# hangelwen/miR-PREFeR

Hardware: AMD Instinct MI355X
Metric: precursor windows folded+filtered/sec (L=300) (higher is better)
Workload: dtype int16/int32 (energies in 0.01 kcal/mol)

## Files before the change

mir-prefer_amd/csrc/fold_lds_common.h:

```cpp
#pragma once
#include <hip/hip_runtime.h>
#include <type_traits>
#include <cstdio>
#include "fold_epilogue.h"
#include "fold185_device.h"

namespace mirp {

#define LNT 1024
#define LNT2 512
#define LCAP 352
#define LDMAX 300
#define LSPAN 300
#define I16_INF 0x7fff
#define FIN_LIMIT 28000
#define FML_BIAS 31500
#define FML_MAX 1267
#define LSEG 384
#define KEY_BIAS 40000
#define KEY_NONE 0xffffffffu
#define KEY_INF (65535u << 10)
#define OTH_BIAS 2048

struct LdsTables {
    short stack[64];
    short bulge[32];
    short internal_loop[32];
    short mismatchI[200], mismatchH[200], mismatchM[200], mismatch1nI[200], mismatch23I[200];
    unsigned char XB[176];
    unsigned char X1[176];
    short dangle5[40], dangle3[40];
    unsigned char rt2[28];
    short ML_closing, ML_intern, TerminalAU, ninio, MAX_NINIO, pad[3];
};
__host__ __device__ constexpr int xt_pslot(int s) { return s == 3 ? 3 : s == 4 ? 4 : 0; }
__host__ __device__ constexpr int xt_qslot(int s) { return s == 1 ? 1 : s == 3 ? 2 : s == 4 ? 1 : 0; }
__host__ __device__ constexpr int xt_pcode(int sp, int sp_m1) { return xt_pslot(sp) * 25 + sp_m1; }
__host__ __device__ constexpr int xt_qcode(int sq, int sq_p1) { return xt_qslot(sq) * 25 + sq_p1 * 5; }
static_assert(xt_pslot(1) + xt_qslot(4) == 1 && xt_pslot(2) + xt_qslot(3) == 2 && xt_pslot(3) + xt_qslot(2) == 3 && xt_pslot(3) + xt_qslot(4) == 4 &&
              xt_pslot(4) + xt_qslot(1) == 5 && xt_pslot(4) + xt_qslot(3) == 6, "inner-pair table slots");
template <class TAB>
__device__ inline void xt_fill(TAB& T, const FoldParams* __restrict__ P, int tid, int nt) {
    for (int x = tid; x < 175; x += nt) {
        const int slot = x / 25, a = (x % 25) / 5, b = x % 5;
        const int sp = slot == 1 ? 1 : slot == 2 ? 2 : (slot == 3 || slot == 4) ? 3 : 4, sq = slot == 1 ? 4 : slot == 2 ? 3 : slot == 3 ? 2 : slot == 4 ? 4 : slot == 5 ? 1 : 3;
        const int t2 = slot ? rtype_of(pair_type(sp, sq)) : 0;
        int xb = 0, x1 = 0;
        if (t2) {
            const int mi = P->mismatchI[t2][a][b];
            xb = (t2 > 2 ? P->TerminalAU : 0) - mi;
            x1 = P->mismatch1nI[t2][a][b] - mi;
        }
        T.XB[x] = (unsigned char)(xb + P->xb_bias); T.X1[x] = (unsigned char)(x1 + P->x1_bias);
    }
}
#define CSTR 354
static_assert(CSTR == MIRP_RING_CSTR, "FoldParams::ring_rowoff is built for this row stride");
#define MIRP_CK(d) ((d) % 3)
#define CRING_ROWS 33

struct LTab {
    static constexpr bool kTiled = true;
    const short* fml;
    const int* off;
    const short* carch;
    const unsigned short* tb;
    __device__ __forceinline__ int at(int d, int i) const { return off[(i - 1) >> 3] + ((i - 1) & 7) + 8 * (d - 4); }
    __device__ __forceinline__ int TB(int d, int i) const { return tb[at(d, i)]; }
    __device__ __forceinline__ int C(int d, int i) const { int v = carch[at(d, i)]; return v == I16_INF ? INF : v; }
    __device__ __forceinline__ int TBat(int o) const { return tb[o]; }
    __device__ __forceinline__ int Cat(int o) const { int v = carch[o]; return v == I16_INF ? INF : v; }
    __device__ __forceinline__ int Mat(int o) const { const int v = (unsigned short)fml[o]; return v == 65535 ? INF : v - FML_BIAS; }
    __device__ __forceinline__ int M(int d, int i) const {
        if (d < 4) return INF;
        const int v = (unsigned short)fml[at(d, i)];
        return v == 65535 ? INF : v - FML_BIAS;
    }
};

__device__ __forceinline__ int lds_mlstem(const LdsTables& T, const FoldParams* __restrict__ P, int type, int a, int b) {
    int e = T.ML_intern + (type > 2 ? T.TerminalAU : 0);
    if (a >= 0 && b >= 0) e += T.mismatchM[type * 25 + a * 5 + b];
    else if (a >= 0) e += P->dangle5[type][a];
    else if (b >= 0) e += P->dangle3[type][b];
    return e;
}

__device__ __forceinline__ int lds_intloop(const LdsTables& T, const FoldParams* __restrict__ P, int n1, int n2, int type, int type2,
                                           int si1, int sj1, int sp1, int sq1) {
    int nl = n1 > n2 ? n1 : n2, ns = n1 > n2 ? n2 : n1;
// ... 12 lines not shown
               T.mismatch1nI[type2 * 25 + sq1 * 5 + sp1];
    }
    if (ns == 2) {
        if (nl == 2) return P->int22[type][type2][si1][sp1][sq1][sj1];
        if (nl == 3) return T.internal_loop[5] + T.ninio + T.mismatch23I[type * 25 + si1 * 5 + sj1] + T.mismatch23I[type2 * 25 + sq1 * 5 + sp1];
    }
    int x = (nl - ns) * T.ninio;
    return T.internal_loop[nl + ns] + (x < T.MAX_NINIO ? x : T.MAX_NINIO) + T.mismatchI[type * 25 + si1 * 5 + sj1] +
           T.mismatchI[type2 * 25 + sq1 * 5 + sp1];
}

__host__ __device__ constexpr int tri_off(int d, int n) { return 1 + (d - 4) * n - (d * (d - 1) / 2 - 6) + (((d - 4) + (n & 1)) >> 1); }
__host__ __device__ constexpr int tri_len(int d, int n) { return n - d > 0 ? (n - d) + ((n - d) & 1) : 0; }
__host__ __device__ constexpr int tri_len_any(int d, int n) { return (n - d) + ((n - d) & 1); }
__device__ inline void fill_tri_off(int* off, int n) {
    int o = 1;
    for (int d = 4; d <= LDMAX + 1; d++) { off[d] = o; o += tri_len(d, n); }
}

#define ARCH_RB ((LCAP + 7) / 8)
__host__ __device__ constexpr int arch_nd(int b, int n, int dcap) {
    int m = n - 1 - 8 * b;
    if (m > dcap) m = dcap;
    m -= 3;
    return m > 0 ? (m + 7) & ~7 : 0;
}
__host__ __device__ inline int arch_rowblk_off(int b, int n, int dcap) {
    int o = 0;
    for (int x = 0; x < b; x++) o += 8 * arch_nd(x, n, dcap);
    return o;
}

struct LdsLayout {
    unsigned fml, aux, S, seq, pax, qb2, list, tabs, misc, total, fml_bytes, code4;
};
#define CODE_STR 368
__host__ __device__ constexpr unsigned lds_al(unsigned x) { return (x + 15u) & ~15u; }
#define FML_REGION_BYTES (lds_al((tri_off(LDMAX + 1, LCAP) + 2) * 2))
#define POOL_MIN_CAP 1024
#define FRING_STR (LCAP + 2)
#define LDS_TWO_BYTES (80u * 1024u)
template <int MODEL, bool SPARSE = false, bool TWO = false>
__host__ __device__ constexpr LdsLayout lds_layout() {
    static_assert(!TWO || (SPARSE && MODEL == 0), "two windows per CU: candidate-pool pass of the default model only");
    LdsLayout L{};
    unsigned o = 0;
    if (!SPARSE) { L.fml = o; L.fml_bytes = FML_REGION_BYTES; o += L.fml_bytes; }
    L.aux = o; o += lds_al(CRING_ROWS * CSTR * 2 + (MODEL ? 5 : 3) * LCAP * 2 + (SPARSE ? 6 : 5) * LCAP * 4);
    L.S = o; o += lds_al(LCAP + 8);
    L.seq = o; o += lds_al(LCAP + 8);
    if (SPARSE) {
        L.code4 = o; L.qb2 = o; L.pax = o + 4 * CODE_STR; o += 8 * CODE_STR;
    } else {
        L.pax = o; o += CODE_STR;
        L.qb2 = o; o += CODE_STR;
    }
    L.list = o; o += lds_al(3 * LSEG * 4);
    L.tabs = o; o += lds_al((unsigned)sizeof(LdsTables));
    L.misc = o; o += lds_al((48 + ARCH_RB + ((SPARSE && MODEL) ? 48 : 0)) * 4);
    if (SPARSE) { L.fml = o; L.fml_bytes = (TWO ? LDS_TWO_BYTES : 160u * 1024u) - o; o += L.fml_bytes; }
    L.total = o;
    return L;
}
static_assert(lds_layout<0>().total <= 160 * 1024 && lds_layout<1>().total <= 160 * 1024, "fill kernel LDS budget");
static_assert(lds_layout<0, true, true>().total <= LDS_TWO_BYTES, "two workgroups of the candidate-pool pass must fit one CU's 160 KB");
static_assert((lds_layout<0, true, true>().fml_bytes - lds_al(2 * FRING_STR * 2)) / 6 >= 2 * POOL_MIN_CAP, "two-per-CU layout: room for the candidate pool behind the fML ring");

typedef const volatile __attribute__((address_space(3))) unsigned short* lds_vu16;
typedef const volatile __attribute__((address_space(3))) unsigned char* lds_vu8;
typedef const volatile __attribute__((address_space(3))) unsigned* lds_vu32;
#ifndef MIRP_A1_SMALLPACK
#define MIRP_A1_SMALLPACK 10
#endif
typedef unsigned short us2 __attribute__((ext_vector_type(2)));
typedef unsigned char pax_t;
typedef lds_vu8 lds_vpax;
struct A1 {
    const FoldParams* __restrict__ P;
    const LdsTables* T;
    const unsigned char* S;
    const unsigned short* cring;
    const pax_t* pax;
    const unsigned char* qbr;
    const unsigned char* code4 = nullptr;
    int r0, um, n;
    const int* __restrict__ rowtab;
    const unsigned short* rba = nullptr;
    unsigned w_lo = 0, w_hie = 0, w_hio = 0, w_sh = 0;
};

static_assert(CSTR % 2 == 0, "the aligned-dword ring reads need dword-aligned ring rows");
static_assert((CRING_ROWS - 1) * CSTR + (LCAP - 2) + 1 + MAXLOOP + 1 < CRING_ROWS * CSTR + 3 * LCAP, "the ring over-read stays inside the aux region");

template <bool CHECK, int U>
__device__ __forceinline__ void a1_gen_row(const A1& a, const unsigned short* rb, unsigned& bg) {
    if constexpr (!CHECK && U >= 8) {
        lds_vu32 rq = (lds_vu32)(a.rba + a.rowtab[U]);
        constexpr int m1 = (U - 2) >> 1;
        unsigned dw[m1 + 2];
#pragma unroll
        for (int k = 1; k <= m1 + 1; k++) dw[k] = rq[k];
        const unsigned c1024 = 1024u;
#pragma unroll
        for (int m = 1; m <= m1; m++) {
            const unsigned re = __builtin_amdgcn_alignbit(dw[m + 1], dw[m], a.w_sh);
            unsigned e;
            asm("v_mad_u32_u16 %0, %1, %2, %3" : "=v"(e) : "v"(re), "v"(c1024), "s"(a.P->gen_key[U - 6][2 * m]));
            bg = e < bg ? e : bg;
            if (2 * m + 1 <= U - 2) {
                asm("v_mad_u32_u16 %0, %1, %2, %3 op_sel:[1,0,0,0]" : "=v"(e) : "v"(re), "v"(c1024), "s"(a.P->gen_key[U - 6][2 * m + 1]));
                bg = e < bg ? e : bg;
            }
        }
    } else
    if (!CHECK || U <= a.um) {
        lds_vu16 rp = (lds_vu16)(rb + a.rowtab[U]);
        unsigned v[U - 3];
#pragma unroll
        for (int n1 = 2; n1 <= U - 2; n1++) v[n1 - 2] = rp[n1];
#pragma unroll
        for (int n1 = 2; n1 <= U - 2; n1++) {
            const unsigned e = (v[n1 - 2] << 10) + a.P->gen_key[U - 6][n1];
            bg = e < bg ? e : bg;
        }
    }
}
__device__ __forceinline__ unsigned a1_key(unsigned b, int adj) {
    return b >= KEY_INF ? KEY_NONE : ((unsigned)((int)(b >> 10) + adj + KEY_BIAS) << 10) | (b & 1023u);
}
template <bool CHECK, int WD, int U>
__device__ __forceinline__ void a1_gen_row_w(const A1& a, const unsigned short* rb, unsigned& bg) {
    constexpr int nL = (U - WD) / 2, nR = (U + WD + 1) / 2;
    if constexpr (!CHECK && nL < 4 && U >= MIRP_A1_SMALLPACK) {
        lds_vu32 rq = (lds_vu32)(a.rba + a.rowtab[U]);
        constexpr int m1 = (U - 2) >> 1;
        unsigned dw[m1 + 2];
#pragma unroll
        for (int k = 1; k <= m1 + 1; k++) dw[k] = rq[k];
        const unsigned c1024 = 1024u;
#pragma unroll
        for (int m = 1; m <= m1; m++) {
            const unsigned re = __builtin_amdgcn_alignbit(dw[m + 1], dw[m], a.w_sh);
#pragma unroll
            for (int h = 0; h < 2; h++) {
                const int n1 = 2 * m + h, dd = 2 * n1 - U;
                if (n1 <= U - 2) {
                    const unsigned kt = (dd <= -WD || dd >= WD) ? a.P->gen_wing_key[U - 6] : a.P->gen_key[U - 6][n1];
                    unsigned e;
                    if (h) asm("v_mad_u32_u16 %0, %1, %2, %3 op_sel:[1,0,0,0]" : "=v"(e) : "v"(re), "v"(c1024), "s"(kt));
                    else asm("v_mad_u32_u16 %0, %1, %2, %3" : "=v"(e) : "v"(re), "v"(c1024), "s"(kt));
                    bg = e < bg ? e : bg;
                }
            }
        }
    } else
    if constexpr (!CHECK && nL >= 4) {
        lds_vu32 rq = (lds_vu32)(a.rba + a.rowtab[U]);
        constexpr int kL1 = (1 + nL) >> 1, kR0 = nR >> 1, kR1 = (U - 1) >> 1;
        constexpr int m0 = (nL + 1) >> 1, m1 = (nR - 1) >> 1;
        static_assert(m1 + 1 <= kR1, "the centre's realigned dwords lie inside the row's reads");
        unsigned dw[kR1 + 1];
#pragma unroll
        for (int k = 1; k <= kR1; k++) dw[k] = rq[k];
        unsigned re[m1 - m0 + 1];
#pragma unroll
        for (int m = m0; m <= m1; m++) re[m - m0] = __builtin_amdgcn_alignbit(dw[m + 1], dw[m], a.w_sh);
        us2 mm, t;
        { const unsigned f = dw[1] | a.w_lo; __builtin_memcpy(&mm, &f, 4); }
#pragma unroll
        for (int k = 2; k <= kL1; k++) { __builtin_memcpy(&t, &dw[k], 4); mm = __builtin_elementwise_min(mm, t); }
#pragma unroll
        for (int k = kR0; k < kR1; k++) { __builtin_memcpy(&t, &dw[k], 4); mm = __builtin_elementwise_min(mm, t); }
        { const unsigned l = dw[kR1] | ((U & 1) ? a.w_hio : a.w_hie); __builtin_memcpy(&t, &l, 4); mm = __builtin_elementwise_min(mm, t); }
        const unsigned w0 = mm[0], w1 = mm[1], w = w0 < w1 ? w0 : w1;
        { const unsigned k = (w << 10) + a.P->gen_wing_key[U - 6]; bg = k < bg ? k : bg; }
        const unsigned c1024 = 1024u;
#pragma unroll
        for (int n1 = nL + 1; n1 < nR; n1++) {
            unsigned e;
            if (n1 & 1) asm("v_mad_u32_u16 %0, %1, %2, %3 op_sel:[1,0,0,0]" : "=v"(e) : "v"(re[(n1 >> 1) - m0]), "v"(c1024), "s"(a.P->gen_key[U - 6][n1]));
            else asm("v_mad_u32_u16 %0, %1, %2, %3" : "=v"(e) : "v"(re[(n1 >> 1) - m0]), "v"(c1024), "s"(a.P->gen_key[U - 6][n1]));
            bg = e < bg ? e : bg;
        }
    } else
    if (!CHECK || U <= a.um) {
        lds_vu16 rp = (lds_vu16)(rb + a.rowtab[U]);
        unsigned v[U - 3];
#pragma unroll
        for (int n1 = 2; n1 <= U - 2; n1++) v[n1 - 2] = rp[n1];
        unsigned w = 65535u;
        unsigned e[2 * WD];
        int ne = 0;
#pragma unroll
        for (int n1 = 2; n1 <= U - 2; n1++) {
            const int dd = 2 * n1 - U;
            if (dd <= -WD || dd >= WD) w = v[n1 - 2] < w ? v[n1 - 2] : w;
            else e[ne++] = (v[n1 - 2] << 10) + a.P->gen_key[U - 6][n1];
        }
        if (U - 4 >= WD) { const unsigned k = (w << 10) + a.P->gen_wing_key[U - 6]; bg = k < bg ? k : bg; }
#pragma unroll
        for (int k = 0; k < ne; k++) bg = e[k] < bg ? e[k] : bg;
    }
}
template <bool CHECK, int... Us>
__device__ __forceinline__ unsigned a1_generic(const A1& a0, int i, int j, int mm_outer) {
    unsigned bg = KEY_INF;
    const unsigned short* rb = a0.cring + i + 1;
    A1 a = a0;
    if constexpr (!CHECK) {
        const unsigned par = ((unsigned)(size_t)(lds_vu16)rb >> 1) & 1u;
        a.rba = rb - par; a.w_sh = par * 16u;
    }
    (a1_gen_row<CHECK, Us>(a, rb, bg), ...);
    return a1_key(bg, -32768 + mm_outer);
}
template <bool CHECK, int WD, int... Us>
__device__ __forceinline__ unsigned a1_generic_w(const A1& a0, int i, int j, int mm_outer) {
    unsigned bg = KEY_INF;
    const unsigned short* rb = a0.cring + i + 1;
    A1 a = a0;
    if constexpr (!CHECK) {
        const unsigned par = ((unsigned)(size_t)(lds_vu16)rb >> 1) & 1u;
        a.rba = rb - par;
        a.w_lo = par ? 0xffffu : 0u; a.w_hie = par ? 0u : 0xffff0000u; a.w_hio = par ? 0xffff0000u : 0xffffffffu; a.w_sh = par * 16u;
    }
    (a1_gen_row_w<CHECK, WD, Us>(a, rb, bg), ...);
    return a1_key(bg, -32768 + mm_outer);
}

template <bool CHECK, int LO, int HI>
__device__ __forceinline__ void a1_b0(const A1& a, int i, int j, unsigned& best) {
    const unsigned idxp = a.pax[i + 1];
    lds_vu8 ql = (lds_vu8)(a.qbr + (a.n + 2 - j));
    const unsigned short* rb = a.cring + i + 1;
    const unsigned char* xb = a.T->XB;
#pragma unroll
    for (int U = LO; U <= HI; U++) {
        if (!CHECK || U <= a.um) {
            const unsigned idx2 = idxp + ql[U];
            const int x = xb[idx2];
            const unsigned g = rb[((a.r0 - U) & 31) * CSTR];
            const unsigned e = ((g + (unsigned)x) << 10) + a.P->kb0_key[U];
            best = e < best ? e : best;
        }
    }
}
template <bool CHECK, int LO, int HI>
__device__ __forceinline__ void a1_b1(const A1& a, int i, int j, unsigned& best) {
    const unsigned idxq = a.qbr[a.n + 2 - j];
    lds_vpax pl = (lds_vpax)(a.pax + i + 1);
    const unsigned short* rb = a.cring + i + 1;
    const unsigned char* xb = a.T->XB;
#pragma unroll
    for (int U = LO; U <= HI; U++) {
        if (!CHECK || U <= a.um) {
            const unsigned idx2 = idxq + pl[U];
            const int x = xb[idx2];
            const unsigned g = rb[((a.r0 - U) & 31) * CSTR + U];
            const unsigned e = ((g + (unsigned)x) << 10) + a.P->kb1_key[U];
// ... 242 lines not shown
```

mir-prefer_amd/csrc/fold_lds_kernel.hip:

```cpp
#include "fold_lds_common.h"
#ifndef MIRP_CPERIOD0
#define MIRP_CPERIOD0 0
#endif
#ifndef MIRP_CPERIOD1
#define MIRP_CPERIOD1 64
#endif
#define CPOOL_ROUNDS 4

namespace mirp {

template <int MODEL, bool SPARSE, int NT = LNT>
__global__ void __launch_bounds__(NT, 4) fold_lds_kernel(
    const FoldParams* __restrict__ P, const unsigned char* __restrict__ seqs, const long long* __restrict__ offs, const int* __restrict__ win_lens,
    int n_work, int win_base, int span, short* __restrict__ slabs, size_t slab_shorts, int* __restrict__ win_state,
    unsigned int* __restrict__ work_counter, int* __restrict__ fallback_list,
    unsigned int* __restrict__ fallback_count, int max_lines, int ss_stride, MirpFoldLine* __restrict__ out_lines, char* __restrict__ out_ss,
    int* __restrict__ out_nlines, int* __restrict__ out_mfe, int* __restrict__ out_status, int light_clocks_arg, long long* __restrict__ dbg_cycles_arg,
    const int* __restrict__ todo_list, const unsigned int* __restrict__ todo_count, int* __restrict__ dense_list, unsigned int* __restrict__ dense_count) {
    extern __shared__ __align__(16) unsigned char smem[];
    constexpr bool TWO = NT != LNT;
    static_assert(NT == LNT || NT == LNT2, "workgroup size");
    constexpr int NW = NT / 64;
    constexpr LdsLayout LY = lds_layout<MODEL, SPARSE, TWO>();
#ifdef MIRP_DIAG
    const bool light = light_clocks_arg != 0;
    long long* const dbg_cycles = dbg_cycles_arg;
#else
    constexpr bool light = false;
    constexpr long long* dbg_cycles = nullptr;
    (void)light_clocks_arg; (void)dbg_cycles_arg;
#endif
    constexpr int DMLR = MODEL ? 5 : 3;
#define ENT_OUTER(mmo, mm1) ((unsigned)(((mmo) & 1023) | (((mm1) & 1023) << 10)))
    const int tau_s = __builtin_amdgcn_readfirstlane(P->TerminalAU);
    constexpr int GEN_WD = 5;
    long long tA = 0, tB = 0, tS = 0, tE = 0, t0 = 0;
    long long wB = 0, wA1 = 0, wA2 = 0, wW = 0, wt = 0;
    unsigned short* fml = (unsigned short*)(smem + LY.fml);
    unsigned short* cring = (unsigned short*)(smem + LY.aux);
    short* dmlring = (short*)(cring + CRING_ROWS * CSTR);
    int* acc = (int*)(dmlring + DMLR * LCAP);
    constexpr int NACC = SPARSE ? 6 : 5;
    auto mdec_of = [&](int d) -> int* { return acc + (3 + (SPARSE ? d % 3 : (d & 1))) * LCAP; };
    unsigned char* S = smem + LY.S;
    unsigned char* seq = smem + LY.seq;
    pax_t* pax = (pax_t*)(smem + LY.pax);
    unsigned char* qbr = smem + LY.qb2;
    unsigned char* code4 = SPARSE ? smem + LY.code4 : nullptr;
    short* spec = (short*)(cring + 29 * CSTR);
    using list_t = unsigned;
    list_t* list = (list_t*)(smem + LY.list);
    LdsTables& T = *(LdsTables*)(smem + LY.tabs);
    int* misc = (int*)(smem + LY.misc);
    int* lcnt = misc + 16;
    int* rbt = misc + 48;
    const int tid = threadIdx.x, lane = tid & 63;
    const int wave = __builtin_amdgcn_readfirstlane(tid >> 6);
    if (wave < (TWO ? 6 : 12)) __builtin_amdgcn_s_setprio(1);
    const int nc = CSTR;
    auto list_append = [&](int dd, int i, int t, int oi) {
        const unsigned long long bal = __ballot(t != 0);
        if (bal) {
            int base = 0;
            if (lane == 0) base = atomicAdd(&lcnt[dd % 6], (int)__popcll(bal));
            base = __builtin_amdgcn_readfirstlane(base);
            if (t) list[(dd % 3) * LSEG + base + __popcll(bal & ((1ull << lane) - 1ull))] = (list_t)((unsigned)i | ((unsigned)t << 9) | ((unsigned)oi << 12));
        }
    };

    for (int x = tid; x < 64; x += NT) T.stack[x] = (short)min(P->stack[x >> 3][x & 7], (int)I16_INF);
    for (int x = tid; x < 31; x += NT) { T.bulge[x] = (short)min(P->bulge[x], (int)I16_INF); T.internal_loop[x] = (short)min(P->internal_loop[x], (int)I16_INF); }
    for (int x = tid; x < 200; x += NT) {
        int t = x / 25, a = (x % 25) / 5, b = x % 5;
        T.mismatchI[x] = (short)min(P->mismatchI[t][a][b], (int)I16_INF); T.mismatchH[x] = (short)min(P->mismatchH[t][a][b], (int)I16_INF);
        T.mismatchM[x] = (short)P->mismatchM[t][a][b]; T.mismatch1nI[x] = (short)min(P->mismatch1nI[t][a][b], (int)I16_INF);
        T.mismatch23I[x] = (short)min(P->mismatch23I[t][a][b], (int)I16_INF);
    }
    xt_fill(T, P, tid, NT);
    if (tid < 40) { T.dangle5[tid] = (short)P->dangle5[tid / 5][tid % 5]; T.dangle3[tid] = (short)P->dangle3[tid / 5][tid % 5]; }
    if (tid < 25) T.rt2[tid] = (unsigned char)rtype_of(pair_type(tid / 5, tid % 5));
    if (tid == 0) { T.ML_closing = (short)P->ML_closing; T.ML_intern = (short)P->ML_intern; T.TerminalAU = (short)P->TerminalAU; T.ninio = (short)P->ninio; T.MAX_NINIO = (short)P->MAX_NINIO; }
    if constexpr (MODEL != 0) if (tid == 0) misc[4] = 0;
// ... 21 lines not shown
        short* fml_out = carch + slab_shorts;
        unsigned short* tb_out = reinterpret_cast<unsigned short*>(carch + 2 * slab_shorts);
        if (dbg_cycles && tid == 0) t0 = clock64();
        int xki = 0;
        if constexpr (MODEL != 0) {
            if (n >= 1 && n <= LCAP - 2)
                for (int x = tid; x < n; x += NT) { const unsigned u = seqs[o0 + x] & 0xdfu; if (u == 'X' || u == 'K' || u == 'I') misc[4] = 1; }
            __syncthreads();
            xki = misc[4];
            __syncthreads();
            if (tid == 0) misc[4] = 0;
        }
        if (n < 1 || n > LCAP - 2 || xki) {
            if (tid == 0) {
                out_nlines[win] = 0; out_mfe[win] = 0; out_status[win] = 0; win_state[win] = 0;
                if (n >= 1) { unsigned int k = atomicAdd(fallback_count, 1u); fallback_list[k] = win_base + win; }
            }
        } else if (SPARSE && pool_cap < POOL_MIN_CAP) {
            if (tid == 0) { out_nlines[win] = 0; out_mfe[win] = 0; out_status[win] = 0; win_state[win] = 0; dense_list[atomicAdd(dense_count, 1u)] = win; }
        } else {
        const int D = (span - 1 < n - 1) ? span - 1 : n - 1;
        const int Dm = MODEL ? ((span < n - 1) ? span : n - 1) : D;
        for (int x = tid; x <= n + 1; x += NT) {
            unsigned char ch = 0;
            if (x >= 1 && x <= n) {
                ch = seqs[o0 + x - 1];
                if (ch >= 'a' && ch <= 'z') ch -= 32;
                if (ch == 'T') ch = 'U';
            }
            seq[x] = ch;
            S[x] = ch == 'A' ? 1 : ch == 'C' ? 2 : ch == 'G' ? 3 : ch == 'U' ? 4 : 0;
        }
        for (int x = tid; x < DMLR * LCAP; x += NT) dmlring[x] = (short)I16_INF;
        for (int x = tid; x < NACC * LCAP; x += NT) acc[x] = x >= 3 * LCAP ? INF : (int)KEY_NONE;
        if (tid == 0) {
            misc[1] = 0; misc[2] = 0; misc[3] = 0;
            if constexpr (SPARSE && MODEL != 0) for (int x = 0; x < 44; x++) pbits[x] = 0;
            for (int x = 0; x < 6; x++) lcnt[x] = 0;
        }
        if (tid >= 64 && tid < 64 + ARCH_RB) rbt[tid - 64] = arch_rowblk_off(tid - 64, n, span);
        __syncthreads();
        if (tid == 0) { S[0] = S[n]; S[n + 1] = S[1]; }
        for (int x = tid; x <= n; x += NT) {
            short s3 = -32768, s4 = -32768, s6 = -32768;
            if (x >= 1) {
                if (x + 4 <= n)
                    for (int k = 0; k < P->n_tri; k++) { bool m = true; for (int t = 0; t < 5; t++) m = m && (seq[x + t] == (unsigned char)P->tri[k][t]); if (m && s3 == -32768) s3 = (short)P->triE[k]; }
                if (x + 5 <= n)
                    for (int k = 0; k < P->n_tetra; k++) { bool m = true; for (int t = 0; t < 6; t++) m = m && (seq[x + t] == (unsigned char)P->tetra[k][t]); if (m && s4 == -32768) s4 = (short)P->tetraE[k]; }
                if (x + 7 <= n)
                    for (int k = 0; k < P->n_hexa; k++) { bool m = true; for (int t = 0; t < 8; t++) m = m && (seq[x + t] == (unsigned char)P->hexa[k][t]); if (m && s6 == -32768) s6 = (short)P->hexaE[k]; }
            }
            if (MODEL) s4 = s4 == -32768 ? (short)0 : s4;
            spec[x] = s3; spec[nc + x] = s4; spec[2 * nc + x] = s6;
            if (x >= 1) {
                pax[x] = (pax_t)xt_pcode(S[x], x > 1 ? (int)S[x - 1] : 0);
                qbr[n + 1 - x] = (unsigned char)xt_qcode(S[x], x < n ? (int)S[x + 1] : 0);
            }
        }
        for (int dd = 4; dd <= 6 && dd <= D; dd++) {
            int t = 0, oi = 0;
            if (tid < n - dd) {
                t = pair_type(S[tid + 1], S[tid + 1 + dd]);
                const int x = t * 25 + S[tid + 2] * 5 + S[tid + dd];
                oi = ENT_OUTER((int)T.mismatchI[x], (int)T.mismatch1nI[x]);
            }
// ... 242 lines not shown
                    unsigned res = KEY_NONE;
                    int au1 = 0, mmo = 0, mm1 = 0;
                    if (role < 14 || MODEL == 0) {
                        au1 = type > 2 ? tau_s : 0;
                        mmo = ((int)(ent << 10)) >> 22; mm1 = ((int)ent) >> 22;
                    }
                    if (role < 8) {
#define MIRP_GEN(CK)                                                                      \
    switch (role) {                                                                       \
    case 0: res = MIRP_A1G<CK MIRP_A1WD, 30, 23>(a, i, j, mmo); if (CK) a1_i1<CK, 28, 29>(a, i, j, xi); else a1_i1f<28, 29>(a, i, j, xi); break;      \
    case 1: res = MIRP_A1G<CK MIRP_A1WD, 29, 24>(a, i, j, mmo); if (CK) a1_i1<CK, 25, 27>(a, i, j, xi); else a1_i1f<25, 27>(a, i, j, xi); break;      \
    case 2: res = MIRP_A1G<CK MIRP_A1WD, 28, 25>(a, i, j, mmo); if (CK) a1_i0<CK, 26, 29>(a, i, j, xi); else a1_i0f<26, 29>(a, i, j, xi); break;      \
    case 3: res = MIRP_A1G<CK MIRP_A1WD, 27, 26>(a, i, j, mmo); if (CK) a1_b1<CK, 26, 30>(a, i, j, xb); else a1_b1f<26, 30>(a, i, j, xb); break;      \
    case 4: res = MIRP_A1G<CK MIRP_A1WD, MIRP_ROWS4>(a, i, j, mmo); break;                    \
    case 5: res = MIRP_A1G<CK MIRP_A1WD, MIRP_ROWS5>(a, i, j, mmo); break;                    \
    case 6: res = MIRP_A1G<CK MIRP_A1WD, MIRP_ROWS6>(a, i, j, mmo); break;                    \
    default: res = MIRP_A1G<CK MIRP_A1WD, MIRP_ROWS7>(a, i, j, mmo); break;               \
    }
#define MIRP_XGEN(CK)                                                                     \
    switch (role) {                                                                       \
    case 15: rx = MIRP_A1G<CK MIRP_A1WD, MIRP_XROWS15>(a, i, j, mmo); break;                         \
    case 8: rx = MIRP_A1G<CK MIRP_A1WD, MIRP_XROWS8>(a, i, j, mmo); break;                           \
    case 9: rx = MIRP_A1G<CK MIRP_A1WD, MIRP_XROWS9>(a, i, j, mmo); break;                           \
    default: break;                                                                       \
    }
                        unsigned xb = KEY_INF, xi = KEY_INF;
                        if constexpr (MODEL == 0) {
#define MIRP_A1G a1_generic_w
#define MIRP_A1WD , GEN_WD
#define MIRP_ROWS4 22, 17, 12
#define MIRP_ROWS5 21, 18, 11
#define MIRP_ROWS6 20, 16, 13
#define MIRP_ROWS7 19, 15, 14, 6
                            if (a.um >= MAXLOOP) { MIRP_GEN(false) } else { MIRP_GEN(true) }
#undef MIRP_A1G
#undef MIRP_A1WD
#undef MIRP_ROWS4
#undef MIRP_ROWS5
#undef MIRP_ROWS6
#undef MIRP_ROWS7
                        } else {
#define MIRP_A1G a1_generic
#define MIRP_A1WD
#define MIRP_ROWS4 22, 17, 12, 7
#define MIRP_ROWS5 21, 18, 11, 8
#define MIRP_ROWS6 20, 16, 13, 9
#define MIRP_ROWS7 19, 15, 14, 10, 6
                            if (a.um >= MAXLOOP) { MIRP_GEN(false) } else { MIRP_GEN(true) }
#undef MIRP_A1G
#undef MIRP_A1WD
#undef MIRP_ROWS4
#undef MIRP_ROWS5
#undef MIRP_ROWS6
#undef MIRP_ROWS7
                        }
                        if (role < 4) {
                            const unsigned rb = a1_key(xb, -32768 - OTH_BIAS + au1);
                            const unsigned ri = a1_key(xi, -32768 - OTH_BIAS + mm1);
                            res = rb < res ? rb : res;
                            res = ri < res ? ri : res;
                        }
#undef MIRP_GEN
                    } else if (role < 14) {
                        unsigned bb = KEY_INF, bi = KEY_INF;
                        if (a.um >= MAXLOOP) {
                            switch (role) {
                            case 8: a1_b0f<2, 18>(a, i, j, bb); break;
                            case 9: a1_b0f<19, 30>(a, i, j, bb); a1_b1f<2, 6>(a, i, j, bb); break;
                            case 10: a1_b1f<7, 22>(a, i, j, bb); break;
                            case 11: a1_b1f<23, 25>(a, i, j, bb); a1_i0f<3, 15>(a, i, j, bi); break;
                            case 12: a1_i0f<16, 25>(a, i, j, bi); a1_i1f<3, 8>(a, i, j, bi); break;
                            default: a1_i1f<9, 24>(a, i, j, bi); break;
                            }
                        } else {
                            switch (role) {
                            case 8: a1_b0<true, 2, 18>(a, i, j, bb); break;
                            case 9: a1_b0<true, 19, 30>(a, i, j, bb); a1_b1<true, 2, 6>(a, i, j, bb); break;
                            case 10: a1_b1<true, 7, 22>(a, i, j, bb); break;
                            case 11: a1_b1<true, 23, 25>(a, i, j, bb); a1_i0<true, 3, 15>(a, i, j, bi); break;
                            case 12: a1_i0<true, 16, 25>(a, i, j, bi); a1_i1<true, 3, 8>(a, i, j, bi); break;
                            default: a1_i1<true, 9, 24>(a, i, j, bi); break;
                            }
                        }
                        const unsigned rb = a1_key(bb, -32768 - OTH_BIAS + au1);
                        const unsigned ri = a1_key(bi, -32768 - OTH_BIAS + mm1);
                        res = rb < ri ? rb : ri;
                    } else if (a.um >= MAXLOOP) {
                        res = role == 14 ? a1_small14f(a, i, j, type, ahead) : a1_small15f(a, i, j, type);
                    } else {
                        const int si1 = S[i + 1], sj1 = S[j - 1];
                        int ra, ca, rb2, cb2;
                        unsigned ka, kb2;
                        if (role == 14) {
                            a1_small_g<1, 1>(a, i, j, type, si1, sj1, ra, ca); a1_small_g<1, 2>(a, i, j, type, si1, sj1, rb2, cb2);
                            unsigned r00 = KEY_NONE;
                            a1_small<0, 0>(a, i, j, type, si1, sj1, r00); a1_small<0, 1>(a, i, j, type, si1, sj1, res); a1_small<1, 0>(a, i, j, type, si1, sj1, res);
                            if (!ahead) res = r00 < res ? r00 : res;
                            ka = 1 << 5 | 1; kb2 = 1 << 5 | 2;
                        } else {
                            a1_small_g<2, 1>(a, i, j, type, si1, sj1, ra, ca); a1_small_g<2, 2>(a, i, j, type, si1, sj1, rb2, cb2);
                            a1_small<2, 3>(a, i, j, type, si1, sj1, res); a1_small<3, 2>(a, i, j, type, si1, sj1, res);
                            ka = 2 << 5 | 1; kb2 = 2 << 5 | 2;
                        }
                        if (ca < INF) { const unsigned k = ((unsigned)(ra + ca + KEY_BIAS) << 10) | ka; res = k < res ? k : res; }
                        if (cb2 < INF) { const unsigned k = ((unsigned)(rb2 + cb2 + KEY_BIAS) << 10) | kb2; res = k < res ? k : res; }
                    }
                    if constexpr (MODEL == 0) {
                        if (role >= 8) {
                            unsigned rx = KEY_NONE;
#define MIRP_A1G a1_generic_w
#define MIRP_A1WD , GEN_WD
                            if (a.um >= MAXLOOP) { MIRP_XGEN(false) } else { MIRP_XGEN(true) }
#undef MIRP_A1G
#undef MIRP_A1WD
                            res = rx < res ? rx : res;
                        }
                    }
                    if (act && res != KEY_NONE) atomicMin(&ck[i], res);
                }
                if (role == 14 && done > 0) {
                    const bool act = lane < done;
                    const unsigned ent = act ? clist[lane] : (1u | (1u << 9));
                    const int i = ent & 511, type = (ent >> 9) & 7, j = i + d;
                    int r0 = d - 2, um = MAXLOOP;
                    asm volatile("" : "+s"(r0), "+s"(um));
                    a.r0 = r0; a.um = um; a.cring = cring;
                    unsigned res = KEY_NONE;
                    a1_small<0, 0>(a, i, j, type, S[i + 1], S[j - 1], res);
                    if (act && res != KEY_NONE) atomicMin(&ckey[i], res);
                }
                }
                if (dbg_cycles && lane == 0 && wave == 9 && !light) {
                    const int b = nblk < 3 ? nblk : 3;
                    atomicAdd((unsigned long long*)&dbg_cycles[68 + b], (unsigned long long)(clock64() - wt));
                    atomicAdd((unsigned long long*)&dbg_cycles[72 + b], 1ull);
                }
            }
            if (dbg_cycles && lane == 0 && !light) { const long long t = clock64(); wA1 += t - wt; wt = t; }
            if (!swap_order) splits();
        };
        auto phaseB0 = [&](const int d) {
            const int ncell = n - d;
            unsigned* ckey = reinterpret_cast<unsigned*>(acc + MIRP_CK(d) * LCAP);
            int* mdec = mdec_of(d);
            int cbase = 0, cand = 0; unsigned cent = 0, cval = 0;
// ... 252 lines not shown
                    const int at = pre + (int)__popcll(al[r] & ((1ull << lane) - 1ull));
                    poolA[at] = ea[r];
                    if constexpr (MODEL != 0) poolB32[at] = eb[r]; else poolB[at] = (unsigned short)eb[r];
                }
                pre += (int)__popcll(al[r]);
            }
            if (tid == 0) misc[3] = tot;
            sp_snap = __builtin_amdgcn_readfirstlane(tot);
            __syncthreads();
        };
        if (tid < n - 4) {
            const int i = tid + 1, j = i + 4;
            lds_vu8 Sv = (lds_vu8)S;
            pb_si = (int)Sv[i - 1] | ((int)Sv[i] << 3) | ((int)Sv[i + 1] << 6);
            pb_sj = (int)Sv[j - 1] | ((int)Sv[j] << 3) | ((int)Sv[j + 1] << 6) | ((int)Sv[j + 2] << 9) | ((int)Sv[j + 3] << 12);
        }
        if (Dm >= 4) phaseA(4);
        __syncthreads();
        if (dbg_cycles && tid == 0) { long long t = clock64(); tA += t - t0; t0 = t; }
        for (int d = 4; d <= Dm; d++) {
            if constexpr (SPARSE) { constexpr int CP = MODEL ? MIRP_CPERIOD1 : MIRP_CPERIOD0; if (CP > 0 && (d & (CP - 1)) == 0 && d >= 32) compact_pool(d); }
            if (dbg_cycles && lane == 0) wt = clock64();
            if constexpr (MODEL != 0) {
                const unsigned la = (unsigned)(size_t)(__attribute__((address_space(3))) int*)&lcnt[(d + 2) % 6];
                asm volatile("ds_read_b32 %0, %1" : "=v"(lc_pre) : "v"(la) : "memory");
                lc_have = true;
            }
            if constexpr (MODEL == 0) phaseB0(d); else phaseB1(d);
            if (dbg_cycles && lane == 0 && !light) { const long long t = clock64(); wB += t - wt; wt = t; }
            if (d + 1 <= Dm) phaseA(d + 1);
            if (dbg_cycles && lane == 0) { const long long t = clock64(); wA2 += t - wt; wt = t; }
            __syncthreads();
            if (dbg_cycles && lane == 0) { const long long t = clock64(); wW += t - wt; wt = t; }
            if (dbg_cycles && tid == 0 && !light) { long long t = clock64(); tB += t - t0; t0 = t; }
        }
        const int overflow = misc[1];
        __syncthreads();
        if (dbg_cycles && tid == 0) { long long t = clock64(); tE += t - t0; t0 = t; }
        const int pool_over = SPARSE ? misc[2] : 0;
        if (overflow) {
            if (tid == 0) { unsigned int k = atomicAdd(fallback_count, 1u); fallback_list[k] = win_base + win; out_nlines[win] = 0; out_mfe[win] = 0; out_status[win] = 0; win_state[win] = 0; }
        } else if (pool_over) {
            if (tid == 0) { out_nlines[win] = 0; out_mfe[win] = 0; out_status[win] = 0; win_state[win] = 0; dense_list[atomicAdd(dense_count, 1u)] = win; }
        } else {
            if (!TWO && Dm >= 4) {
                constexpr int NGD = (LDMAX + 1 - 4) / 64 + 1;
                for (int rb = wave; 8 * rb + 1 + 4 <= n; rb += NW) {
                    const int dmax_rb = Dm < n - 1 - 8 * rb ? Dm : n - 1 - 8 * rb;
                    short* dst = fml_out + rbt[rb] - 32;
                    unsigned v[NGD][8];
#pragma unroll
                    for (int g = 0; g < NGD; g++) {
                        const int d = 4 + 64 * g + lane;
                        const int o = tri_off(d <= dmax_rb ? d : 4, n) + 8 * rb + 1;
#pragma unroll
                        for (int k = 0; k < 8; k++) v[g][k] = fml[o + k];
                    }
#pragma unroll
                    for (int g = 0; g < NGD; g++) {
                        const int d = 4 + 64 * g + lane;
                        if (d <= dmax_rb) {
                            uint4 w;
                            w.x = v[g][0] | v[g][1] << 16; w.y = v[g][2] | v[g][3] << 16; w.z = v[g][4] | v[g][5] << 16; w.w = v[g][6] | v[g][7] << 16;
                            *reinterpret_cast<uint4*>(dst + 8 * d) = w;
                        }
                    }
                }
            }
            if (tid == 0) win_state[win] = 1;
        }
        }
        __syncthreads();
    }
    if (dbg_cycles && lane == 0) {
        atomicAdd((unsigned long long*)&dbg_cycles[4 + wave * 4 + 0], (unsigned long long)wB); atomicAdd((unsigned long long*)&dbg_cycles[4 + wave * 4 + 1], (unsigned long long)wA1);
        atomicAdd((unsigned long long*)&dbg_cycles[4 + wave * 4 + 2], (unsigned long long)wA2); atomicAdd((unsigned long long*)&dbg_cycles[4 + wave * 4 + 3], (unsigned long long)wW);
    }
    if (dbg_cycles && tid == 0) {
        atomicAdd((unsigned long long*)&dbg_cycles[0], (unsigned long long)tS); atomicAdd((unsigned long long*)&dbg_cycles[1], (unsigned long long)tA);
        atomicAdd((unsigned long long*)&dbg_cycles[2], (unsigned long long)tB); atomicAdd((unsigned long long*)&dbg_cycles[3], (unsigned long long)tE);
    }
}

#ifndef ENT
#define ENT 256
#endif
#ifndef MIRP_EPI_WGS
#define MIRP_EPI_WGS 8
#endif
__global__ void __launch_bounds__(ENT, MIRP_EPI_WGS) fold_lds_epilogue_kernel(
    const FoldParams* __restrict__ P, const unsigned char* __restrict__ seqs, const long long* __restrict__ offs, const int* __restrict__ win_lens,
    int n_work, int span, const short* __restrict__ slabs, size_t slab_shorts, const int* __restrict__ win_state, unsigned int* __restrict__ work_counter,
    int max_lines, int ss_stride, MirpFoldLine* __restrict__ out_lines, char* __restrict__ out_ss, int* __restrict__ out_nlines,
    int* __restrict__ out_mfe, int* __restrict__ out_status) {
    extern __shared__ __align__(16) unsigned char smem[];
    const int nc = LCAP + 8;
    int* f3 = (int*)smem;
    int* starts = f3 + nc;
    int* lens = starts + max_lines;
    int* btstk = lens + max_lines;
    int* misc = btstk + (ENT / 64) * 3 * BT_STACK;
    int* off = misc + 16;
    short* spec = (short*)(off + LDMAX + 2);
    unsigned char* S = (unsigned char*)(spec + 3 * nc);
    unsigned char* seq = S + nc;
    char* btbuf = (char*)(seq + nc);
    EpiTables* EP = (EpiTables*)(smem + ((((size_t)(btbuf - (char*)smem) + (ENT / 64) * nc) + 15) & ~(size_t)15));
    short* xtab = (short*)(EP + 1);
    unsigned char* pq2 = (unsigned char*)(xtab + XTAB_N);
    short* ppart = (short*)(pq2 + nc);
    const int tid = threadIdx.x;
    fill_epi_tables(EP, P, tid, ENT);
    fill_ext_table(xtab, P, tid, ENT);
// ... 250 lines not shown
```

mir-prefer_amd/csrc/fold_params.h:

```cpp
#pragma once
#include <stdint.h>

#define MIRP_TURN 3
#define MIRP_MAXLOOP 30
#define MIRP_INF 10000000
#define MIRP_RING_CSTR 354
#define MIRP_HP_MAX 3104

struct alignas(16) FoldParams {
    unsigned gen_key[25][32];
    unsigned kb0_key[31];
    unsigned kb1_key[31];
    unsigned k1n0_key[31];
    unsigned k1n1_key[31];
    unsigned gen_wing_key[25];
    int gen_wing_d;
    int xb_bias, x1_bias;
    int ring_rowoff[32][32];
    int stack[8][8];
    int bulge[31];
    int internal_loop[31];
    int mismatchI[8][5][5];
    int mismatchH[8][5][5];
    int mismatchM[8][5][5];
    int mismatch1nI[8][5][5];
    int mismatch23I[8][5][5];
    int mismatchExt[8][5][5];
    int dangle5[8][5];
    int dangle3[8][5];
    int hairpinE[MIRP_HP_MAX];
    int tetraE[32], triE[2], hexaE[4];
    char tetra[32][8];
    char tri[2][8];
    char hexa[4][12];
    int ML_closing, ML_intern, TerminalAU, ninio, MAX_NINIO;
    int n_tri, n_tetra, n_hexa;
    alignas(16) unsigned gen_key2[25][32];
    alignas(16) unsigned gen_keyt[25][4];
    int int11[8][8][5][5];
// ... 29 lines not shown
```

mir-prefer_amd/csrc/mirp_api.cpp:

```cpp
#include <hip/hip_runtime.h>
#include <algorithm>
#include <cstdio>
#include <cstdlib>
#include <cstring>
#include <string>
#include <vector>
#include "mirp_internal.h"

#define MIRP_ABI_VERSION 17
#define MIRP_NMAX 3096

#include "mirp_ctx.h"
#include "mirp_fasta.h"

extern "C" int mirp_abi_version(void) { return MIRP_ABI_VERSION; }

extern "C" void mirp_destroy(mirp_ctx* c);

extern "C" int mirp_create(int device, mirp_ctx** out) {
    if (!out) return -1;
    *out = nullptr;
    int ndev = 0;
    if (hipGetDeviceCount(&ndev) != hipSuccess || ndev <= 0) return -3;
    if (device < 0 || device >= ndev) return -4;
// ... 332 lines not shown
            const int grid = std::min(nb, c->n_cu);
            const int grid_epi = std::min(nb, c->n_cu * 8);
            while ((int)c->fold_ev.size() < 3 * (n_sub + 1)) { hipEvent_t ev; HIPCHK(c, hipEventCreate(&ev)); c->fold_ev.push_back(ev); }
            hipEvent_t* ev3 = &c->fold_ev[3 * n_sub];
            HIPCHK(c, hipEventRecord(ev3[0], c->stream));
            hipError_t e = mirp::launch_fold_lds(c->stream, m185 ? 1 : 0, grid, grid_epi, m185 ? c->d_params185l : c->d_params, d_seqs, d_offs + b0, d_lens ? d_lens + b0 : nullptr, nb, b0, span,
                                                 (short*)c->carch.p, slab, (int*)c->wstate.p, ctl, (int*)c->flist.p, ctl + 4, max_lines, stride,
                                                 d_lines + (size_t)b0 * max_lines, d_ss + (size_t)b0 * max_lines * stride, d_nlines + b0, d_mfe + b0,
                                                 d_status + b0, light_clocks, dbg_cycles, ev3[1], (int*)c->dlist.p, c->fold_dense);
            if (e != hipSuccess) return fail(c, -2, std::string("fold LDS kernel launch failed: ") + hipGetErrorString(e));
            HIPCHK(c, hipEventRecord(ev3[2], c->stream));
            n_sub++;
        }
        unsigned int nfb2[2] = {0, 0};
        HIPCHK(c, hipMemcpyAsync(nfb2, ctl + 4, 8, hipMemcpyDeviceToHost, c->stream));
        HIPCHK(c, hipStreamSynchronize(c->stream));
        const unsigned int nfb = nfb2[0];
        c->last_fallback = nfb;
        c->last_dense = nfb2[1];
        c->fold_kernel_ms[0] = c->fold_kernel_ms[1] = 0;
        for (int k = 0; k < n_sub; k++) {
            float a = 0, b = 0;
            (void)hipEventElapsedTime(&a, c->fold_ev[3 * k], c->fold_ev[3 * k + 1]);
            (void)hipEventElapsedTime(&b, c->fold_ev[3 * k + 1], c->fold_ev[3 * k + 2]);
            c->fold_kernel_ms[0] += a; c->fold_kernel_ms[1] += b;
        }
#ifdef MIRP_DIAG
        if (const char* dump = std::getenv("MIRP_FOLD_DUMP")) {
            std::vector<short> h(3 * slab);
            HIPCHK(c, hipMemcpy(h.data(), c->carch.p, 6 * slab, hipMemcpyDeviceToHost));
            if (FILE* f = std::fopen(dump, "wb")) { std::fwrite(h.data(), 2, h.size(), f); std::fclose(f); }
        }
        if (dbg_cycles) {
            long long cyc[4 + 64 + 8];
            HIPCHK(c, hipMemcpy(cyc, dbg_cycles, sizeof(cyc), hipMemcpyDeviceToHost));
            std::fprintf(stderr, "[mirp fold clocks] windows=%d setup=%lld fillA=%lld fillB=%lld writeout=%lld (sum over workgroups, s_memtime ticks)\n", n_work,
                         cyc[0], cyc[1], cyc[2], cyc[3]);
            for (int w = 0; w < 16; w++)
                std::fprintf(stderr, "[mirp fold clocks] wave %2d: phaseB=%lld interior=%lld splits=%lld barrier=%lld\n", w, cyc[4 + 4 * w], cyc[5 + 4 * w], cyc[6 + 4 * w],
                             cyc[7 + 4 * w]);
            for (int b = 0; b < 4; b++)
                std::fprintf(stderr, "[mirp fold clocks] wave 9, diagonals with %d%s blocks: %lld, interior ticks %lld\n", b, b == 3 ? "+" : "", cyc[72 + b], cyc[68 + b]);
            mirp::fold_lds_epi_clocks_print();
        }
#endif
        if (nfb == 0) return 0;
        work_list = (const int*)c->flist.p;
        n_generic = (int)nfb;
    }
    return run_generic(work_list, n_generic);
}

extern "C" int mirp_collapse_reads(mirp_ctx* c, const char* path, const char* prefix, const char* out_path, int32_t hash_bits, int64_t* n_reads,
                                   int64_t* n_unique, double seconds[6]) {
    if (!c) return -1;
    if (!path || !prefix || !out_path || hash_bits < 1 || hash_bits > 64) return fail(c, -1, "mirp_collapse_reads: bad argument");
    double sec[6] = {0, 0, 0, 0, 0, 0};
    HIPCHK(c, hipSetDevice(c->device));
    double t = mirp::now();
    FILE* f = std::fopen(path, "rb");
    if (!f) return fail(c, -8, std::string("cannot open ") + path);
    fseeko(f, 0, SEEK_END);
    const long long n = (long long)ftello(f);
    fseeko(f, 0, SEEK_SET);
    char* text = (char*)std::malloc((size_t)n + 1);
    if (!text) { std::fclose(f); return fail(c, -7, "host allocation failed (collapse: text)"); }
    const size_t got = n > 0 ? std::fread(text, 1, (size_t)n, f) : 0;
    std::fclose(f);
    if ((long long)got != n) { std::free(text); return fail(c, -8, std::string("cannot read ") + path); }
    sec[0] = mirp::now() - t;
    char* out = nullptr;
    long long out_len = 0, nr = 0, nu = 0, bad = -1;
    const int rc = mirp_device_collapse_reads(c, text, n, prefix, hash_bits, &out, &out_len, &nr, &nu, &bad, sec);
    if (rc == -9) {
        char msg[160];
// ... 19 lines not shown
```

Before: 344,100.

## Drop bounds-checked ramp-up path via padded ring rows and hoist row keys into SGPRs

The ring row stride and pair-code copy stride are widened, the ring is pre-filled with INF, and the spec buffer gets its own region in the two-per-CU layout. This lets the early diagonals, where fewer than MAXLOOP rows exist, use the unchecked fast interior-loop generators instead of the bounds-checked ones. Separately, per-row key constants and row offsets are hoisted into scalar registers ahead of the generic row loops and pinned with empty asm. The cost is extra LDS footprint and possible SGPR pressure. Debug timing counters for ramp-up intervals are also added.

```diff
diff --git a/mir-prefer_amd/csrc/fold_lds_common.h b/mir-prefer_amd/csrc/fold_lds_common.h
--- a/mir-prefer_amd/csrc/fold_lds_common.h
+++ b/mir-prefer_amd/csrc/fold_lds_common.h
@@ -1,6 +1,7 @@
 #pragma once
 #include <hip/hip_runtime.h>
 #include <type_traits>
+#include <tuple>
 #include <cstdio>
 #include "fold_epilogue.h"
 #include "fold185_device.h"
@@ -54,8 +55,7 @@
         T.XB[x] = (unsigned char)(xb + P->xb_bias); T.X1[x] = (unsigned char)(x1 + P->x1_bias);
     }
 }
-#define CSTR 354
-static_assert(CSTR == MIRP_RING_CSTR, "FoldParams::ring_rowoff is built for this row stride");
+#define CSTR MIRP_RING_CSTR
 #define MIRP_CK(d) ((d) % 3)
 #define CRING_ROWS 33
 
@@ -134,11 +134,12 @@
 }
 
 struct LdsLayout {
-    unsigned fml, aux, S, seq, pax, qb2, list, tabs, misc, total, fml_bytes, code4;
+    unsigned fml, aux, S, seq, pax, qb2, list, tabs, misc, total, fml_bytes, code4, spec;
 };
-#define CODE_STR 368
+#define CODE_STR 384
+static_assert(CODE_STR % 16 == 0 && (LCAP - 2) - 5 + MAXLOOP + 3 < CODE_STR, "pair-code reads of the first diagonals stay inside their copy");
 __host__ __device__ constexpr unsigned lds_al(unsigned x) { return (x + 15u) & ~15u; }
-#define FML_REGION_BYTES (lds_al((tri_off(LDMAX + 1, LCAP) + 2) * 2))
+#define FML_REGION_BYTES (lds_al((tri_off(LDMAX + 1, LCAP - 2) + 2) * 2))
 #define POOL_MIN_CAP 1024
 #define FRING_STR (LCAP + 2)
 #define LDS_TWO_BYTES (80u * 1024u)
@@ -160,6 +161,7 @@
     L.list = o; o += lds_al(3 * LSEG * 4);
     L.tabs = o; o += lds_al((unsigned)sizeof(LdsTables));
     L.misc = o; o += lds_al((48 + ARCH_RB + ((SPARSE && MODEL) ? 48 : 0)) * 4);
+    if (TWO) { L.spec = o; o += lds_al(3 * CSTR * 2); }
     if (SPARSE) { L.fml = o; L.fml_bytes = (TWO ? LDS_TWO_BYTES : 160u * 1024u) - o; o += L.fml_bytes; }
     L.total = o;
     return L;
@@ -193,6 +195,9 @@
 
 static_assert(CSTR % 2 == 0, "the aligned-dword ring reads need dword-aligned ring rows");
 static_assert((CRING_ROWS - 1) * CSTR + (LCAP - 2) + 1 + MAXLOOP + 1 < CRING_ROWS * CSTR + 3 * LCAP, "the ring over-read stays inside the aux region");
+#ifndef MIRP_RAMP_OLD_STRIDE
+static_assert((LCAP - 2) - 6 + 1 + MAXLOOP + 1 < CSTR, "ramp-up diagonals: a lane's ring reads stay inside their row");
+#endif
 
 template <bool CHECK, int U>
 __device__ __forceinline__ void a1_gen_row(const A1& a, const unsigned short* rb, unsigned& bg) {
@@ -230,9 +235,42 @@
 __device__ __forceinline__ unsigned a1_key(unsigned b, int adj) {
     return b >= KEY_INF ? KEY_NONE : ((unsigned)((int)(b >> 10) + adj + KEY_BIAS) << 10) | (b & 1023u);
 }
+#ifndef MIRP_A1_HOIST
+#define MIRP_A1_HOIST 1
+#endif
+template <int WD, int U>
+struct A1RowK {
+    static constexpr int nL = (U - WD) / 2, nR = (U + WD + 1) / 2;
+    static constexpr bool kWinged = nL >= 4;
+    static constexpr int NC = kWinged ? nR - nL - 1 : 1;
+    static_assert(NC <= 5, "a1_rows_pin takes five centre keys");
+    int ro;
+    unsigned kw, kc[NC];
+};
+template <bool ON, int WD, int U>
+__device__ __forceinline__ A1RowK<WD, U> a1_row_k(const A1& a) {
+    A1RowK<WD, U> k{};
+    if constexpr (ON && A1RowK<WD, U>::kWinged) {
+        k.ro = a.rowtab[U];
+        k.kw = a.P->gen_wing_key[U - 6];
+#pragma unroll
+        for (int c = 0; c < A1RowK<WD, U>::NC; c++) k.kc[c] = a.P->gen_key[U - 6][A1RowK<WD, U>::nL + 1 + c];
+    }
+    return k;
+}
+template <int WD, int U>
+__device__ __forceinline__ void a1_row_pin(A1RowK<WD, U>& k) {
+    if constexpr (A1RowK<WD, U>::kWinged) {
+        constexpr int NC = A1RowK<WD, U>::NC;
+        if constexpr (NC == 5) asm volatile("" : "+s"(k.ro), "+s"(k.kw), "+s"(k.kc[0]), "+s"(k.kc[1]), "+s"(k.kc[2]), "+s"(k.kc[3]), "+s"(k.kc[4]));
+        else if constexpr (NC == 4) asm volatile("" : "+s"(k.ro), "+s"(k.kw), "+s"(k.kc[0]), "+s"(k.kc[1]), "+s"(k.kc[2]), "+s"(k.kc[3]));
+        else asm volatile("" : "+s"(k.ro), "+s"(k.kw), "+s"(k.kc[0]));
+    }
+}
 template <bool CHECK, int WD, int U>
-__device__ __forceinline__ void a1_gen_row_w(const A1& a, const unsigned short* rb, unsigned& bg) {
+__device__ __forceinline__ void a1_gen_row_w(const A1& a, const unsigned short* rb, unsigned& bg, const A1RowK<WD, U>& rk) {
     constexpr int nL = (U - WD) / 2, nR = (U + WD + 1) / 2;
+    constexpr bool HOIST = !CHECK && MIRP_A1_HOIST != 0;
     if constexpr (!CHECK && nL < 4 && U >= MIRP_A1_SMALLPACK) {
         lds_vu32 rq = (lds_vu32)(a.rba + a.rowtab[U]);
         constexpr int m1 = (U - 2) >> 1;
@@ -257,7 +295,7 @@
         }
     } else
     if constexpr (!CHECK && nL >= 4) {
-        lds_vu32 rq = (lds_vu32)(a.rba + a.rowtab[U]);
+        lds_vu32 rq = (lds_vu32)(a.rba + (HOIST ? rk.ro : a.rowtab[U]));
         constexpr int kL1 = (1 + nL) >> 1, kR0 = nR >> 1, kR1 = (U - 1) >> 1;
         constexpr int m0 = (nL + 1) >> 1, m1 = (nR - 1) >> 1;
         static_assert(m1 + 1 <= kR1, "the centre's realigned dwords lie inside the row's reads");
@@ -275,13 +313,14 @@
         for (int k = kR0; k < kR1; k++) { __builtin_memcpy(&t, &dw[k], 4); mm = __builtin_elementwise_min(mm, t); }
         { const unsigned l = dw[kR1] | ((U & 1) ? a.w_hio : a.w_hie); __builtin_memcpy(&t, &l, 4); mm = __builtin_elementwise_min(mm, t); }
         const unsigned w0 = mm[0], w1 = mm[1], w = w0 < w1 ? w0 : w1;
-        { const unsigned k = (w << 10) + a.P->gen_wing_key[U - 6]; bg = k < bg ? k : bg; }
+        { const unsigned k = (w << 10) + (HOIST ? rk.kw : a.P->gen_wing_key[U - 6]); bg = k < bg ? k : bg; }
         const unsigned c1024 = 1024u;
 #pragma unroll
         for (int n1 = nL + 1; n1 < nR; n1++) {
             unsigned e;
-            if (n1 & 1) asm("v_mad_u32_u16 %0, %1, %2, %3 op_sel:[1,0,0,0]" : "=v"(e) : "v"(re[(n1 >> 1) - m0]), "v"(c1024), "s"(a.P->gen_key[U - 6][n1]));
-            else asm("v_mad_u32_u16 %0, %1, %2, %3" : "=v"(e) : "v"(re[(n1 >> 1) - m0]), "v"(c1024), "s"(a.P->gen_key[U - 6][n1]));
+            const unsigned kt = HOIST ? rk.kc[n1 - nL - 1] : a.P->gen_key[U - 6][n1];
+            if (n1 & 1) asm("v_mad_u32_u16 %0, %1, %2, %3 op_sel:[1,0,0,0]" : "=v"(e) : "v"(re[(n1 >> 1) - m0]), "v"(c1024), "s"(kt));
+            else asm("v_mad_u32_u16 %0, %1, %2, %3" : "=v"(e) : "v"(re[(n1 >> 1) - m0]), "v"(c1024), "s"(kt));
             bg = e < bg ? e : bg;
         }
     } else
@@ -326,7 +365,10 @@
         a.rba = rb - par;
         a.w_lo = par ? 0xffffu : 0u; a.w_hie = par ? 0u : 0xffff0000u; a.w_hio = par ? 0xffff0000u : 0xffffffffu; a.w_sh = par * 16u;
     }
-    (a1_gen_row_w<CHECK, WD, Us>(a, rb, bg), ...);
+    constexpr bool HOIST = !CHECK && MIRP_A1_HOIST != 0;
+    std::tuple<A1RowK<WD, Us>...> ks{a1_row_k<HOIST, WD, Us>(a)...};
+    if constexpr (HOIST) (a1_row_pin<WD, Us>(std::get<A1RowK<WD, Us>>(ks)), ...);
+    (a1_gen_row_w<CHECK, WD, Us>(a, rb, bg, std::get<A1RowK<WD, Us>>(ks)), ...);
     return a1_key(bg, -32768 + mm_outer);
 }
 
diff --git a/mir-prefer_amd/csrc/fold_lds_kernel.hip b/mir-prefer_amd/csrc/fold_lds_kernel.hip
--- a/mir-prefer_amd/csrc/fold_lds_kernel.hip
+++ b/mir-prefer_amd/csrc/fold_lds_kernel.hip
@@ -35,6 +35,7 @@
     const int tau_s = __builtin_amdgcn_readfirstlane(P->TerminalAU);
     constexpr int GEN_WD = 5;
     long long tA = 0, tB = 0, tS = 0, tE = 0, t0 = 0;
+    long long tR = 0, nR = 0, nB = 0;
     long long wB = 0, wA1 = 0, wA2 = 0, wW = 0, wt = 0;
     unsigned short* fml = (unsigned short*)(smem + LY.fml);
     unsigned short* cring = (unsigned short*)(smem + LY.aux);
@@ -47,7 +48,12 @@
     pax_t* pax = (pax_t*)(smem + LY.pax);
     unsigned char* qbr = smem + LY.qb2;
     unsigned char* code4 = SPARSE ? smem + LY.code4 : nullptr;
-    short* spec = (short*)(cring + 29 * CSTR);
+#ifdef MIRP_RAMP_CHECKED
+    constexpr bool RAMPF = false;
+#else
+    constexpr bool RAMPF = TWO;
+#endif
+    short* spec = RAMPF ? (short*)(smem + LY.spec) : (short*)(cring + 29 * CSTR);
     using list_t = unsigned;
     list_t* list = (list_t*)(smem + LY.list);
     LdsTables& T = *(LdsTables*)(smem + LY.tabs);
@@ -135,6 +141,11 @@
             S[x] = ch == 'A' ? 1 : ch == 'C' ? 2 : ch == 'G' ? 3 : ch == 'U' ? 4 : 0;
         }
         for (int x = tid; x < DMLR * LCAP; x += NT) dmlring[x] = (short)I16_INF;
+        if constexpr (RAMPF) {
+            static_assert((CRING_ROWS * CSTR) % 2 == 0, "ring initialisation by dwords");
+            unsigned* cr32 = reinterpret_cast<unsigned*>(cring);
+            for (int x = tid; x < CRING_ROWS * CSTR / 2; x += NT) cr32[x] = 0xffffffffu;
+        }
         for (int x = tid; x < NACC * LCAP; x += NT) acc[x] = x >= 3 * LCAP ? INF : (int)KEY_NONE;
         if (tid == 0) {
             misc[1] = 0; misc[2] = 0; misc[3] = 0;
@@ -443,7 +454,7 @@
 #define MIRP_ROWS5 21, 18, 11
 #define MIRP_ROWS6 20, 16, 13
 #define MIRP_ROWS7 19, 15, 14, 6
-                            if (a.um >= MAXLOOP) { MIRP_GEN(false) } else { MIRP_GEN(true) }
+                            if (RAMPF || a.um >= MAXLOOP) { MIRP_GEN(false) } else { MIRP_GEN(true) }
 #undef MIRP_A1G
 #undef MIRP_A1WD
 #undef MIRP_ROWS4
@@ -457,7 +468,7 @@
 #define MIRP_ROWS5 21, 18, 11, 8
 #define MIRP_ROWS6 20, 16, 13, 9
 #define MIRP_ROWS7 19, 15, 14, 10, 6
-                            if (a.um >= MAXLOOP) { MIRP_GEN(false) } else { MIRP_GEN(true) }
+                            if (RAMPF || a.um >= MAXLOOP) { MIRP_GEN(false) } else { MIRP_GEN(true) }
 #undef MIRP_A1G
 #undef MIRP_A1WD
 #undef MIRP_ROWS4
@@ -474,7 +485,7 @@
 #undef MIRP_GEN
                     } else if (role < 14) {
                         unsigned bb = KEY_INF, bi = KEY_INF;
-                        if (a.um >= MAXLOOP) {
+                        if (RAMPF || a.um >= MAXLOOP) {
                             switch (role) {
                             case 8: a1_b0f<2, 18>(a, i, j, bb); break;
                             case 9: a1_b0f<19, 30>(a, i, j, bb); a1_b1f<2, 6>(a, i, j, bb); break;
@@ -496,7 +507,7 @@
                         const unsigned rb = a1_key(bb, -32768 - OTH_BIAS + au1);
                         const unsigned ri = a1_key(bi, -32768 - OTH_BIAS + mm1);
                         res = rb < ri ? rb : ri;
-                    } else if (a.um >= MAXLOOP) {
+                    } else if (RAMPF || a.um >= MAXLOOP) {
                         res = role == 14 ? a1_small14f(a, i, j, type, ahead) : a1_small15f(a, i, j, type);
                     } else {
                         const int si1 = S[i + 1], sj1 = S[j - 1];
@@ -521,7 +532,7 @@
                             unsigned rx = KEY_NONE;
 #define MIRP_A1G a1_generic_w
 #define MIRP_A1WD , GEN_WD
-                            if (a.um >= MAXLOOP) { MIRP_XGEN(false) } else { MIRP_XGEN(true) }
+                            if (RAMPF || a.um >= MAXLOOP) { MIRP_XGEN(false) } else { MIRP_XGEN(true) }
 #undef MIRP_A1G
 #undef MIRP_A1WD
                             res = rx < res ? rx : res;
@@ -840,7 +851,12 @@
             if (dbg_cycles && lane == 0) { const long long t = clock64(); wA2 += t - wt; wt = t; }
             __syncthreads();
             if (dbg_cycles && lane == 0) { const long long t = clock64(); wW += t - wt; wt = t; }
-            if (dbg_cycles && tid == 0 && !light) { long long t = clock64(); tB += t - t0; t0 = t; }
+            if (dbg_cycles && tid == 0 && !light) {
+                long long t = clock64();
+                tB += t - t0; nB++;
+                if (d + 1 >= 6 && d + 1 <= D && d + 1 - 2 - (TURN + 1) < MAXLOOP) { tR += t - t0; nR++; }
+                t0 = t;
+            }
         }
         const int overflow = misc[1];
         __syncthreads();
@@ -887,6 +903,8 @@
     if (dbg_cycles && tid == 0) {
         atomicAdd((unsigned long long*)&dbg_cycles[0], (unsigned long long)tS); atomicAdd((unsigned long long*)&dbg_cycles[1], (unsigned long long)tA);
         atomicAdd((unsigned long long*)&dbg_cycles[2], (unsigned long long)tB); atomicAdd((unsigned long long*)&dbg_cycles[3], (unsigned long long)tE);
+        atomicAdd((unsigned long long*)&dbg_cycles[76], (unsigned long long)tR); atomicAdd((unsigned long long*)&dbg_cycles[77], (unsigned long long)nR);
+        atomicAdd((unsigned long long*)&dbg_cycles[78], (unsigned long long)nB);
     }
 }
 
diff --git a/mir-prefer_amd/csrc/fold_params.h b/mir-prefer_amd/csrc/fold_params.h
--- a/mir-prefer_amd/csrc/fold_params.h
+++ b/mir-prefer_amd/csrc/fold_params.h
@@ -4,7 +4,9 @@
 #define MIRP_TURN 3
 #define MIRP_MAXLOOP 30
 #define MIRP_INF 10000000
-#define MIRP_RING_CSTR 354
+#ifndef MIRP_RING_CSTR
+#define MIRP_RING_CSTR 378
+#endif
 #define MIRP_HP_MAX 3104
 
 struct alignas(16) FoldParams {
diff --git a/mir-prefer_amd/csrc/mirp_api.cpp b/mir-prefer_amd/csrc/mirp_api.cpp
--- a/mir-prefer_amd/csrc/mirp_api.cpp
+++ b/mir-prefer_amd/csrc/mirp_api.cpp
@@ -388,7 +388,7 @@
             if (FILE* f = std::fopen(dump, "wb")) { std::fwrite(h.data(), 2, h.size(), f); std::fclose(f); }
         }
         if (dbg_cycles) {
-            long long cyc[4 + 64 + 8];
+            long long cyc[4 + 64 + 8 + 3];
             HIPCHK(c, hipMemcpy(cyc, dbg_cycles, sizeof(cyc), hipMemcpyDeviceToHost));
             std::fprintf(stderr, "[mirp fold clocks] windows=%d setup=%lld fillA=%lld fillB=%lld writeout=%lld (sum over workgroups, s_memtime ticks)\n", n_work,
                          cyc[0], cyc[1], cyc[2], cyc[3]);
@@ -397,6 +397,8 @@
                              cyc[7 + 4 * w]);
             for (int b = 0; b < 4; b++)
                 std::fprintf(stderr, "[mirp fold clocks] wave 9, diagonals with %d%s blocks: %lld, interior ticks %lld\n", b, b == 3 ? "+" : "", cyc[72 + b], cyc[68 + b]);
+            std::fprintf(stderr, "[mirp fold clocks] ramp-up intervals (interior loops with um < MAXLOOP): %lld of %lld intervals, %lld of fillB=%lld ticks (%.1f %%)\n", cyc[77], cyc[78],
+                         cyc[76], cyc[2], cyc[2] ? 100.0 * (double)cyc[76] / (double)cyc[2] : 0.0);
             mirp::fold_lds_epi_clocks_print();
         }
 #endif
```

New measurement: 350,000 (median of 6 runs). +1.7%, better.
